# jgkellymit/GENIE-SMEM

Measured on NVIDIA B200. Metric: SMEM reads/sec (BWA-SMEM; LUT/RMI under methods), higher is better.
Workload: dtype u32

## Files before the change

genie_smem_b200/csrc/fm_core.cuh:

```cuda
#pragma once
#include <stdint.h>

#if defined(__CUDACC__)
#define GSM_HD __host__ __device__ __forceinline__
#else
#define GSM_HD inline
#endif

namespace gsm {

struct U4 {
    uint32_t x, y, z, w;
};

struct Half {
    uint32_t c0, c1;
    uint32_t l0, l1, l2;
    uint32_t h0, h1, h2;
};

GSM_HD uint32_t popc32(uint32_t v) {
#if defined(__CUDA_ARCH__)
    return (uint32_t)__popc(v);
#else
    return (uint32_t)__builtin_popcount(v);
#endif
}

GSM_HD void split192(uint32_t p, uint32_t& bucket, uint32_t& r) {
#if defined(__CUDA_ARCH__)
    bucket = __umulhi(p >> 6, 0xAAAAAAABu) >> 1;
#else
    bucket = (p >> 6) / 3u;
#endif
    r = p - bucket * 192u;
}

GSM_HD uint32_t mask_low(uint32_t n) {
#if defined(__CUDA_ARCH__)
    uint32_t m;
    asm("bmsk.clamp.b32 %0, %1, %2;" : "=r"(m) : "r"(0u), "r"(n));
    return m;
#else
    return n >= 32u ? 0xFFFFFFFFu : ((1u << n) - 1u);
#endif
}

GSM_HD uint32_t clamp32(int v) { return (uint32_t)(v < 0 ? 0 : (v > 32 ? 32 : v)); }

struct SymK {
    uint32_t fl, fh;
    uint32_t X, Y;
    uint32_t nz;
};

GSM_HD SymK sym_consts(uint32_t c) {
    SymK k;
    k.fl = 0u - ((c & 1u) ^ 1u);
    k.fh = 0u - (((c >> 1) & 1u) ^ 1u);
    k.X = 0u - (c >> 1);
    k.Y = 0u - (c & (c >> 1));
    k.nz = 0u - (uint32_t)(c != 0u);
    return k;
}

GSM_HD uint32_t half_counts(const Half& v, uint32_t r, const SymK& k, uint32_t g) {
    const int n = (int)r - 96 * (int)g;
    const uint32_t m0 = mask_low(clamp32(n)), m1 = mask_low(clamp32(n - 32)), m2 = mask_low(clamp32(n - 64));
    const uint32_t eq = popc32((v.l0 ^ k.fl) & (v.h0 ^ k.fh) & m0) + popc32((v.l1 ^ k.fl) & (v.h1 ^ k.fh) & m1) +
                        popc32((v.l2 ^ k.fl) & (v.h2 ^ k.fh) & m2);
    const uint32_t lt = popc32(((~v.h0 & (~v.l0 | k.X)) | (~v.l0 & k.Y)) & m0 & k.nz) +
                        popc32(((~v.h1 & (~v.l1 | k.X)) | (~v.l1 & k.Y)) & m1 & k.nz) +
                        popc32(((~v.h2 & (~v.l2 | k.X)) | (~v.l2 & k.Y)) & m2 & k.nz);
    return eq | (lt << 8);
}

GSM_HD void half_header(const Half& v, uint32_t c, uint32_t g, uint32_t& h_eq, uint32_t& h_lt) {
    const uint32_t mine = (c >> 1) == g ? ((c & 1u) ? v.c1 : v.c0) : 0u;
    const uint32_t lt0 = (c >= 1u ? v.c0 : 0u) + (c >= 2u ? v.c1 : 0u);
    const uint32_t lt1 = c == 3u ? v.c0 : 0u;
    h_eq = mine;
    h_lt = g == 0u ? lt0 : lt1;
}

struct StepOut {
    uint32_t lo_new, cnt_new, lt_add;
};

GSM_HD StepOut finish_step(uint32_t eq0, uint32_t eq1, uint32_t ltd, uint32_t P0, uint32_t P1, uint32_t c, uint32_t Cc,
                           uint32_t primary) {
    const uint32_t a0 = P0 > primary ? 1u : 0u;
    const uint32_t a1 = P1 > primary ? 1u : 0u;
    const uint32_t inrange = a1 - a0;
    const uint32_t isA = c == 0u ? 1u : 0u;
    StepOut o;
    o.lo_new = Cc + eq0 - (isA & a0);
    o.cnt_new = (eq1 - eq0) - (isA & inrange);
    o.lt_add = isA ? inrange : ltd;
    return o;
}

GSM_HD void bucket_masks(const Half& h0, const Half& h1, const SymK& k, uint32_t (&E)[6], uint32_t (&T)[6]) {
    const uint32_t L[6] = {h0.l0, h0.l1, h0.l2, h1.l0, h1.l1, h1.l2}, H[6] = {h0.h0, h0.h1, h0.h2, h1.h0, h1.h1, h1.h2};
#if defined(__CUDA_ARCH__)
#pragma unroll
#endif
    for (int w = 0; w < 6; ++w) {
        E[w] = (L[w] ^ k.fl) & (H[w] ^ k.fh);
        T[w] = ((~H[w] & (~L[w] | k.X)) | (~L[w] & k.Y)) & k.nz;
    }
}

GSM_HD uint32_t bucket_counts(const uint32_t (&E)[6], const uint32_t (&T)[6], uint32_t r) {
    uint32_t eq = 0, lt = 0;
#if defined(__CUDA_ARCH__)
#pragma unroll
#endif
    for (int w = 0; w < 6; ++w) {
        const uint32_t m = mask_low(clamp32((int)r - 32 * w));
        eq += popc32(E[w] & m);
        lt += popc32(T[w] & m);
    }
    return eq | (lt << 16);
}

template <typename LoadHalf>
GSM_HD StepOut step_single(LoadHalf load, uint32_t P0, uint32_t P1, uint32_t c, uint32_t Cc, uint32_t primary) {
    const SymK k = sym_consts(c);
    uint32_t b0, r0, b1, r1;
    split192(P0, b0, r0);
    split192(P1, b1, r1);
    uint32_t E[6], T[6];
    const Half a0 = load((uint64_t)b0 * 2), a1 = load((uint64_t)b0 * 2 + 1);
    bucket_masks(a0, a1, k, E, T);
    const uint32_t acc0 = bucket_counts(E, T, r0);
    uint32_t e0, l0, e1, l1;
    half_header(a0, c, 0u, e0, l0);
    half_header(a1, c, 1u, e1, l1);
    const uint32_t eq0 = e0 + e1 + (acc0 & 0xFFFFu), lt0 = l0 + l1 + (acc0 >> 16);
    uint32_t eq1, lt1;
    if (b1 == b0) {
        const uint32_t acc1 = bucket_counts(E, T, r1);
        eq1 = e0 + e1 + (acc1 & 0xFFFFu); lt1 = l0 + l1 + (acc1 >> 16);
    } else {
        const Half c0 = load((uint64_t)b1 * 2), c1 = load((uint64_t)b1 * 2 + 1);
        bucket_masks(c0, c1, k, E, T);
        const uint32_t acc1 = bucket_counts(E, T, r1);
        half_header(c0, c, 0u, e0, l0);
        half_header(c1, c, 1u, e1, l1);
        eq1 = e0 + e1 + (acc1 & 0xFFFFu); lt1 = l0 + l1 + (acc1 >> 16);
    }
    return finish_step(eq0, eq1, lt1 - lt0, P0, P1, c, Cc, primary);
}

template <typename LoadHalf>
GSM_HD uint32_t lf_single(LoadHalf load, uint32_t r, const uint32_t* C, uint32_t primary) {
    uint32_t b, off;
    split192(r, b, off);
    const Half h0 = load((uint64_t)b * 2), h1 = load((uint64_t)b * 2 + 1);
    const uint32_t g = off >= 96u ? 1u : 0u, o = off - 96u * g;
    const Half& hs = g ? h1 : h0;
    const uint32_t lw = o < 32u ? hs.l0 : (o < 64u ? hs.l1 : hs.l2);
    const uint32_t hw = o < 32u ? hs.h0 : (o < 64u ? hs.h1 : hs.h2);
    const uint32_t c = ((lw >> (o & 31u)) & 1u) | (((hw >> (o & 31u)) & 1u) << 1);
    const SymK k = sym_consts(c);
    uint32_t e0, l0, e1, l1;
    half_header(h0, c, 0u, e0, l0);
    half_header(h1, c, 1u, e1, l1);
    const uint32_t acc = half_counts(h0, off, k, 0u) + half_counts(h1, off, k, 1u);
    uint32_t rank = e0 + e1 + (acc & 0xFFu);
    if (c == 0u && r > primary) rank -= 1u;
    return C[c] + rank;
}

GSM_HD uint32_t base_msb(const uint32_t* words, uint32_t pos) { return (words[pos >> 4] >> (30u - 2u * (pos & 15u))) & 3u; }

template <typename LoadW>
GSM_HD uint64_t kmer_code(LoadW load, uint64_t p, uint32_t K) {
    uint64_t w = p >> 4;
    uint32_t sh = 2u * (uint32_t)(p & 15u);
    uint64_t hi = ((uint64_t)load(w) << 32) | (uint64_t)load(w + 1);
    uint64_t v = hi << sh;
    if (sh) v |= (uint64_t)load(w + 2) >> (32u - sh);
    return v >> (64u - 2u * K);
}

}
```

genie_smem_b200/csrc/index_device.cu:

```cuda
#include <cuda_runtime.h>

#include <cub/block/block_reduce.cuh>
#include <cub/block/block_scan.cuh>
#include <cub/device/device_radix_sort.cuh>

#include <algorithm>
#include <cstdint>
#include <cstring>
#include <string>

#include "../../include/genie_smem.h"
#include "fm_core.cuh"
#include "host_common.hpp"

namespace gsm {

#define GSM_CUDA(call)                                                                          \
    do {                                                                                        \
        cudaError_t e__ = (call);                                                               \
        if (e__ != cudaSuccess)                                                                 \
            return fail(GSM_E_CUDA, std::string(#call) + ": " + cudaGetErrorString(e__));       \
    } while (0)

namespace {
// ... 137 lines not shown
            if (u) {
                const unsigned long long o = carry_s + eo;
                out_keys[o] = (unsigned long long)head << 32;
                out_vals[o] = start;
                out_pos[o] = row;
            }
        }
        carry_m = max(carry_m, am);
        carry_s += as;
        __syncthreads();
    }
}

__global__ void __launch_bounds__(BT) k_round_keys(unsigned long long* keys, const uint32_t* vals, const uint32_t* rank, uint64_t m, uint64_t h,
                                                   uint64_t N) {
    const uint64_t k = (uint64_t)blockIdx.x * BT + threadIdx.x;
    if (k >= m) return;
    const uint64_t p = (uint64_t)vals[k] + h;
    uint32_t r;
    if (p <= N) r = rank[p];
    else r = (p - N) <= VIRT ? VIRT - (uint32_t)(p - N) : 0u;
    keys[k] |= (unsigned long long)r;
}

__global__ void __launch_bounds__(BT) k_bwt_planes(const uint32_t* sa1, const uint32_t* text, uint64_t n_rows, uint64_t n_buckets, uint32_t* buckets,
                                                   uint4* bucket_cnt, uint32_t* primary) {
    const uint32_t lane = threadIdx.x & 31u;
    const uint64_t warp0 = ((uint64_t)blockIdx.x * BT + threadIdx.x) >> 5;
    const uint64_t n_warps = ((uint64_t)gridDim.x * BT) >> 5;
    for (uint64_t b = warp0; b < n_buckets; b += n_warps) {
        uint32_t c0 = 0, c1 = 0, c2 = 0, c3 = 0;
        uint32_t* w = buckets + b * 16;
#pragma unroll
        for (int g = 0; g < 2; ++g)
#pragma unroll
            for (int mth = 0; mth < 3; ++mth) {
                const uint64_t r = b * GSM_BUCKET_SYMS + 96 * g + 32 * mth + lane;
                const bool valid = r < n_rows;
                uint32_t c = 0;
                if (valid) {
                    const uint32_t s1 = __ldg(sa1 + r);
                    if (s1 == 1u) *primary = (uint32_t)r;
                    else c = text_base(text, (uint64_t)s1 - 2u);
                }
                const uint32_t lo = __ballot_sync(0xFFFFFFFFu, valid && (c & 1u));
                const uint32_t hi = __ballot_sync(0xFFFFFFFFu, valid && (c >> 1));
                const uint32_t vm = __ballot_sync(0xFFFFFFFFu, valid);
                const uint32_t n3 = __popc(lo & hi), n2 = __popc(hi & ~lo), n1 = __popc(lo & ~hi);
                c3 += n3; c2 += n2; c1 += n1; c0 += __popc(vm) - n1 - n2 - n3;
                if (lane == 0) {
                    w[8 * g + 2 + mth] = lo;
                    w[8 * g + 5 + mth] = hi;
                }
            }
        if (lane == 0) bucket_cnt[b] = make_uint4(c0, c1, c2, c3);
    }
}

struct Add4 {
    __device__ __forceinline__ uint4 operator()(const uint4& a, const uint4& b) const { return make_uint4(a.x + b.x, a.y + b.y, a.z + b.z, a.w + b.w); }
};

__global__ void __launch_bounds__(BT) k_cnt_reduce(const uint4* cnt, uint64_t n, uint4* tile_sum) {
    using Reduce = cub::BlockReduce<uint4, BT>;
    __shared__ typename Reduce::TempStorage tmp;
    const uint64_t t0 = (uint64_t)blockIdx.x * TILE;
    uint4 acc = make_uint4(0, 0, 0, 0);
    for (int s = 0; s < SUBTILES; ++s) {
        const uint64_t k = t0 + (uint64_t)s * BT + threadIdx.x;
        if (k < n) acc = Add4()(acc, cnt[k]);
    }
    acc = Reduce(tmp).Reduce(acc, Add4());
    if (threadIdx.x == 0) tile_sum[blockIdx.x] = acc;
}

__global__ void __launch_bounds__(1024) k_cnt_top(uint4* tile_sum, uint64_t n_tiles, uint4* total) {
    using Scan = cub::BlockScan<uint4, 1024>;
    __shared__ typename Scan::TempStorage tmp;
    uint4 carry = make_uint4(0, 0, 0, 0);
    for (uint64_t base = 0; base < n_tiles; base += 1024) {
        const uint64_t t = base + threadIdx.x;
        const uint4 v = t < n_tiles ? tile_sum[t] : make_uint4(0, 0, 0, 0);
        uint4 ex, agg;
        Scan(tmp).ExclusiveScan(v, ex, make_uint4(0, 0, 0, 0), Add4(), agg);
        if (t < n_tiles) tile_sum[t] = Add4()(ex, carry);
        carry = Add4()(carry, agg);
        __syncthreads();
    }
    if (threadIdx.x == 0) *total = carry;
}

__global__ void __launch_bounds__(BT) k_cnt_apply(const uint4* cnt, uint64_t n, const uint4* tile_pre, uint32_t* buckets) {
    using Scan = cub::BlockScan<uint4, BT>;
    __shared__ typename Scan::TempStorage tmp;
    const uint64_t t0 = (uint64_t)blockIdx.x * TILE;
    uint4 carry = tile_pre[blockIdx.x];
    for (int s = 0; s < SUBTILES; ++s) {
        const uint64_t k = t0 + (uint64_t)s * BT + threadIdx.x;
        const uint4 v = k < n ? cnt[k] : make_uint4(0, 0, 0, 0);
        uint4 ex, agg;
        Scan(tmp).ExclusiveScan(v, ex, make_uint4(0, 0, 0, 0), Add4(), agg);
        if (k < n) {
            const uint4 p = Add4()(ex, carry);
            uint32_t* w = buckets + k * 16;
            w[0] = p.x; w[1] = p.y; w[8] = p.z; w[9] = p.w;
        }
        carry = Add4()(carry, agg);
        __syncthreads();
    }
}

struct Carve {
    uint8_t* base;
    uint64_t off = 0;
    explicit Carve(void* b) : base((uint8_t*)b) {}
    template <typename T>
    T* take(uint64_t count) {
        off = (off + 255) & ~255ull;
        T* p = base ? (T*)(base + off) : nullptr;
        off += count * sizeof(T);
        return p;
    }
};

struct Plan {
    unsigned long long *k0, *k1, *tile_off, *scalars;
    uint32_t *v0, *v1, *p0, *p1, *rank, *rtext, *tile_max, *tile_cnt;
    uint4 *bucket_cnt, *cnt_tiles;
    void* cub_tmp;
    uint64_t cub_bytes, total;
};

uint64_t cub_sort_bytes(uint64_t n) {
    size_t bytes = 0;
    cub::DoubleBuffer<unsigned long long> dk(nullptr, nullptr);
    cub::DoubleBuffer<uint32_t> dv(nullptr, nullptr);
    cub::DeviceRadixSort::SortPairs(nullptr, bytes, dk, dv, (uint64_t)n, 0, 64, (cudaStream_t)0);
    return (uint64_t)bytes;
// ... 180 lines not shown
```

genie_smem_b200/csrc/index_host.cpp:

```cpp
#include <algorithm>
#include <cstdint>
#include <cstdio>
#include <cstdlib>
#include <cstring>
#include <new>
#include <string>
#include <thread>
#include <vector>

#include "../../include/genie_smem.h"
#include "host_common.hpp"

namespace gsm {

thread_local std::string g_last_error;

int fail(int code, const std::string& msg) {
    g_last_error = msg;
    return code;
}

namespace {

template <typename Ch>
// ... 79 lines not shown
        } else {
            for (int32_t i = 0; i < n1; ++i) SA1[s1[i]] = i;
        }

        buckets(true);
        for (int32_t i = 1, j = 0; i < n; ++i)
            if (is_lms(i)) s1[j++] = i;
        for (int32_t i = 0; i < n1; ++i) SA1[i] = s1[SA1[i]];
        std::fill(SA + n1, SA + n, -1);
        for (int32_t i = n1 - 1; i >= 0; --i) {
            int32_t j = SA[i];
            SA[i] = -1;
            SA[--bkt[s[j]]] = j;
        }
        induce_l();
        induce_s();
    }
};

}

void suffix_sort(const uint8_t* sym, int32_t* SA, int32_t n) {
    Sais<uint8_t> top;
    top.s = sym; top.SA = SA; top.n = n; top.K = 5;
    top.run();
}

void pack_buckets(const uint8_t* bwt, uint64_t n, std::vector<uint32_t>& out) {
    uint64_t nb = n / GSM_BUCKET_SYMS + 1;
    out.assign(nb * 16, 0);
    uint32_t run[4] = {0, 0, 0, 0};
    for (uint64_t b = 0; b < nb; ++b) {
        uint32_t* w = &out[b * 16];
        w[0] = run[0]; w[1] = run[1]; w[8] = run[2]; w[9] = run[3];
        uint64_t base = b * GSM_BUCKET_SYMS;
        for (int g = 0; g < 2; ++g)
            for (int m = 0; m < 3; ++m) {
                uint32_t lo = 0, hi = 0;
                for (int t = 0; t < 32; ++t) {
                    uint64_t r = base + 96 * g + 32 * m + t;
                    if (r >= n) break;
                    uint32_t c = bwt[r];
                    run[c]++;
                    lo |= (c & 1u) << t;
                    hi |= (c >> 1) << t;
                }
                w[8 * g + 2 + m] = lo;
                w[8 * g + 5 + m] = hi;
            }
    }
}

}

using namespace gsm;

struct gsm_index {
    uint64_t n_bases = 0;
    uint64_t n = 0;
    std::vector<uint8_t> codes;
    std::vector<int32_t> sa0;
    std::vector<uint32_t> fwd, rev;
    uint32_t count[4] = {0, 0, 0, 0};
    uint32_t C[5] = {0, 0, 0, 0, 0};
    uint32_t primary_fwd = 0, primary_rev = 0;
    bool has_rev = false;
};

static int decode_bases(const char* bases, uint64_t n_bases, std::vector<uint8_t>& codes, uint32_t count[4]) {
    static int8_t map[256];
    static bool init = false;
    if (!init) {
        memset(map, -1, sizeof(map));
        map[(int)'A'] = 0; map[(int)'C'] = 1; map[(int)'G'] = 2; map[(int)'T'] = 3;
        init = true;
    }
    codes.resize(n_bases);
    for (uint64_t i = 0; i < n_bases; ++i) {
        int8_t c = map[(uint8_t)bases[i]];
        if (c < 0) return fail(GSM_E_INVALID, "non-ACGT base at offset " + std::to_string(i));
        codes[i] = (uint8_t)c;
        count[c]++;
// ... 208 lines not shown
```

genie_smem_b200/csrc/sweep_device.cuh:

```cuda
#pragma once
#include <cuda_runtime.h>

#include "sweep_logic.cuh"

namespace gsm {

constexpr int SWEEP_THREADS = 128;
constexpr int SWEEP_LPR = 2;
constexpr int SWEEP_GROUPS = SWEEP_THREADS / SWEEP_LPR;
constexpr int SWEEP_CAP = 12;
constexpr int SWEEP_MIN_BLOCKS = 8;

constexpr uint32_t MEMS_ORDERED = 0x80000000u;
constexpr uint32_t MEMS_PICKED = 0x40000000u;
constexpr uint32_t MEMS_COUNT = 0x3FFFFFFFu;

struct SweepArgs {
    const uint4* fwd;
    const uint4* rev;
    IndexMeta meta;
    const uint4* reads;
    const uint32_t* chunk_off;
    const uint32_t* len;
    uint32_t n_reads;
// ... 4 lines not shown
    uint32_t seed_K;
    uint4* mem_pool;
    unsigned long long mem_cap;
    uint32_t* mem_off;
    uint32_t* mem_cnt;
    uint4* scratch;
    unsigned long long* counters;
    const uint32_t* sa;
    const uint32_t* text;
    uint32_t n_bases;
};

extern __shared__ uint4 g_sweep_smem[];

__device__ __forceinline__ Half ldg_half(const uint4* halves_base, size_t half_index) {
    Half h;
    asm volatile("ld.global.nc.v8.u32 {%0,%1,%2,%3,%4,%5,%6,%7}, [%8];"
                 : "=r"(h.c0), "=r"(h.c1), "=r"(h.l0), "=r"(h.l1), "=r"(h.l2), "=r"(h.h0), "=r"(h.h1), "=r"(h.h2)
                 : "l"(halves_base + half_index * 2));
    return h;
}

__device__ __forceinline__ StepOut pair_step(const uint4* __restrict__ bk, uint32_t P0, uint32_t P1, uint32_t ch, uint32_t Cc,
                                             uint32_t primary, uint32_t g, bool active) {
    constexpr uint32_t FULLM = 0xFFFFFFFFu;
    uint32_t b0, r0, b1, r1;
    split192(P0, b0, r0);
    split192(P1, b1, r1);
    Half v0 = Half{0, 0, 0, 0, 0, 0, 0, 0}, v1;
    if (active) v0 = ldg_half(bk, (size_t)b0 * 2 + g);
    v1 = v0;
    if (active && b1 != b0) v1 = ldg_half(bk, (size_t)b1 * 2 + g);
    const SymK k = sym_consts(ch);
    uint32_t packed = half_counts(v0, r0, k, g) | (half_counts(v1, r1, k, g) << 16);
    uint32_t he0, hl0, he1, hl1;
    half_header(v0, ch, g, he0, hl0);
    half_header(v1, ch, g, he1, hl1);
    uint32_t A = he0, B = he1, D = hl1 - hl0;
    packed += __shfl_xor_sync(FULLM, packed, 1);
    A += __shfl_xor_sync(FULLM, A, 1);
    B += __shfl_xor_sync(FULLM, B, 1);
    D += __shfl_xor_sync(FULLM, D, 1);
    const uint32_t eq0 = A + (packed & 0xFFu);
    const uint32_t eq1 = B + ((packed >> 16) & 0xFFu);
    const uint32_t ltd = D + ((packed >> 24) & 0xFFu) - ((packed >> 8) & 0xFFu);
    return finish_step(eq0, eq1, ltd, P0, P1, ch, Cc, primary);
}

__device__ __forceinline__ uint4 ldg_seed(const uint4* p) {
    uint4 v;
    asm volatile("ld.global.nc.v4.u32 {%0,%1,%2,%3}, [%4];" : "=r"(v.x), "=r"(v.y), "=r"(v.z), "=r"(v.w) : "l"(p));
    return v;
}

__device__ __forceinline__ uint32_t spread4(uint32_t x) { return ((x * 0x01004010u) | (x >> 6)) & 0x03030303u; }

struct DevSweepCtx {
    const SweepArgs& a;
    uint32_t cand0;
    uint32_t bytes0;
    uint32_t words0;
    uint4* stage;
    uint4* spill;
    uint32_t g, gmask, gbase;

    __device__ __forceinline__ bool fetch(uint32_t& rid, uint32_t& L) {
        unsigned long long r = 0;
        if (g == 0) r = atomicAdd(&a.counters[3], 1ull);
        r = __shfl_sync(gmask, r, gbase);
        if (r >= a.n_reads) return false;
        rid = (uint32_t)r;
        L = __ldg(a.len + rid);
        const uint32_t off = __ldg(a.chunk_off + rid);
        const uint32_t nch = (L + 63u) >> 6;
        uint4* dst = g_sweep_smem + (bytes0 >> 4);
        __syncwarp(gmask);
        for (uint32_t c = g; c < nch; c += SWEEP_LPR) {
            const uint4 v = __ldg(a.reads + (size_t)off + c);
            g_sweep_smem[(words0 >> 2) + c] = v;
// ... 52 lines not shown
    const uint32_t pair_in_block = threadIdx.x >> 1;
    const uint32_t pair_u4 = SWEEP_CAP + a.read_u4 + a.pack_u4;
    const uint32_t p0 = pair_in_block * pair_u4;
    const size_t gp = (size_t)blockIdx.x * SWEEP_GROUPS + pair_in_block;
    DevSweepCtx ctx{a, p0, (p0 + SWEEP_CAP) * 16u, (p0 + SWEEP_CAP + a.read_u4) * 4u, a.scratch + gp * 2 * a.max_len,
                    a.scratch + gp * 2 * a.max_len + a.max_len, g, 3u << (lane & ~1u), lane & ~1u};
    Sweeper<DevSweepCtx> sw;
    for (;;) {
        const bool need = sw.next(ctx, a.meta);
        if (!__any_sync(0xFFFFFFFFu, need)) break;
        const bool is_seed = need && sw.pending_seed();
        const bool is_step = need && !is_seed;
        uint4 se = make_uint4(0u, 0u, 0u, 0u);
        if (is_seed) se = ldg_seed(a.seed_tab + sw.P0);
        const bool rev = sw.on_reverse();
        const StepOut r = pair_step(rev ? a.rev : a.fwd, sw.P0, sw.P0 + sw.cnt, sw.ch, a.meta.C[sw.ch & 3u],
                                    rev ? a.meta.prim_r : a.meta.prim_f, g, is_step);
        if (is_step) sw.consume(ctx, a.meta, r);
        else if (is_seed) sw.consume_seed(ctx, a.meta, SeedEntry{se.x, se.y, se.z, se.w});
    }
}

constexpr int SWEEP1_THREADS = 128;
constexpr int SWEEP1_CAP = 8;
constexpr int SWEEP1_MIN_BLOCKS = 7;

struct LanePartial {
    uint32_t eq0, lt0;
    bool have;
};

template <bool PAIRED>
__device__ __forceinline__ bool lane_step(const uint4* __restrict__ fwd, const uint4* __restrict__ rev, bool use_rev, uint32_t P0, uint32_t P1,
                                          uint32_t ch, uint32_t Cc, uint32_t primary, bool active, LanePartial& part, StepOut& out) {
    constexpr uint32_t FULLM = 0xFFFFFFFFu;
    uint32_t b0, r0, b1, r1;
    split192(P0, b0, r0);
    split192(P1, b1, r1);
    const bool second = part.have;
    const uint32_t b = second ? b1 : b0;
    Half a0 = Half{0, 0, 0, 0, 0, 0, 0, 0}, a1 = a0;
    if (PAIRED) {
        const uint32_t g = threadIdx.x & 1u;
        const uint32_t mine = (active ? 1u : 0u) | (use_rev ? 2u : 0u);
        const uint32_t pb = __shfl_xor_sync(FULLM, b, 1);
        const uint32_t theirs = __shfl_xor_sync(FULLM, mine, 1);
#pragma unroll
        for (uint32_t r = 0; r < 2u; ++r) {
            const bool own = g == r;
            const uint32_t bb = own ? b : pb, fl = own ? mine : theirs;
            Half h = Half{0, 0, 0, 0, 0, 0, 0, 0};
            if (fl & 1u) h = ldg_half((fl & 2u) ? rev : fwd, (size_t)bb * 2 + (own ? 0u : 1u));
            Half o;
            o.c0 = __shfl_xor_sync(FULLM, h.c0, 1); o.c1 = __shfl_xor_sync(FULLM, h.c1, 1);
            o.l0 = __shfl_xor_sync(FULLM, h.l0, 1); o.l1 = __shfl_xor_sync(FULLM, h.l1, 1); o.l2 = __shfl_xor_sync(FULLM, h.l2, 1);
            o.h0 = __shfl_xor_sync(FULLM, h.h0, 1); o.h1 = __shfl_xor_sync(FULLM, h.h1, 1); o.h2 = __shfl_xor_sync(FULLM, h.h2, 1);
            if (own) { a0 = h; a1 = o; }
        }
    } else if (active) {
        const uint4* bk = use_rev ? rev : fwd;
        a0 = ldg_half(bk, (size_t)b * 2);
        a1 = ldg_half(bk, (size_t)b * 2 + 1);
    }
    const SymK k = sym_consts(ch);
    uint32_t E[6], T[6];
    bucket_masks(a0, a1, k, E, T);
    const uint32_t accA = bucket_counts(E, T, second ? r1 : r0);
    const uint32_t accB = bucket_counts(E, T, r1);
    uint32_t e0, l0, e1, l1;
    half_header(a0, ch, 0u, e0, l0);
    half_header(a1, ch, 1u, e1, l1);
    const uint32_t he = e0 + e1, hl = l0 + l1;
    if (!active) return false;
    if (!second && b1 != b0) {
        part.eq0 = he + (accA & 0xFFFFu);
        part.lt0 = hl + (accA >> 16);
        part.have = true;
        return false;
    }
    const uint32_t eq0 = second ? part.eq0 : he + (accA & 0xFFFFu);
    const uint32_t eq1 = he + ((second ? accA : accB) & 0xFFFFu);
    const uint32_t ltd = second ? hl + (accA >> 16) - part.lt0 : (accB >> 16) - (accA >> 16);
    part.have = false;
    out = finish_step(eq0, eq1, ltd, P0, P1, ch, Cc, primary);
    return true;
}

__device__ __noinline__ void hand_over_long(const uint4* sp, uint32_t n, uint4* dst) {
    constexpr uint32_t FULLM = 0xFFFFFFFFu;
    const uint32_t lane = threadIdx.x & 31u;
    uint4 v0 = make_uint4(0u, 0u, 0u, 0u), v1 = v0;
    if (lane < n) v0 = __ldcg(sp + lane);
    if (lane + 32u < n) v1 = __ldcg(sp + lane + 32u);
    const uint32_t prev0 = __shfl_up_sync(FULLM, v0.w, 1);
    const uint32_t last0 = __shfl_sync(FULLM, v0.w, 31);
    uint32_t prev1 = __shfl_up_sync(FULLM, v1.w, 1);
    if (lane == 0u) prev1 = last0;
    const unsigned long long heads =
        (unsigned long long)__ballot_sync(FULLM, lane < n && (lane == 0u || v0.w != prev0)) |
        ((unsigned long long)__ballot_sync(FULLM, lane + 32u < n && v1.w != prev1) << 32);
    uint32_t* seg = reinterpret_cast<uint32_t*>(dst);
#pragma unroll
    for (int half = 0; half < 2; ++half) {
        const uint32_t x = lane + 32u * half;
        if (x < n) {
            const uint4 v = half ? v1 : v0;
            const unsigned long long upto = heads & (~0ull >> (63u - x));
            const uint32_t s0 = 63u - (uint32_t)__clzll((long long)upto);
            const unsigned long long above = x == 63u ? 0ull : heads & (~0ull << (x + 1u));
            const uint32_t s1 = above ? (uint32_t)__ffsll((long long)above) - 1u : n;
            const uint32_t d = s0 + (s1 - 1u - x);
            seg[d] = v.x; seg[n + d] = v.y; seg[2u * n + d] = v.z; seg[3u * n + d] = v.w;
        }
    }
}
// ... 122 lines not shown
            } else if (n <= SOA_MAX) {
                hand_over_long(sp, n, a.mem_pool + off);
            } else {
                for (uint32_t k = lane; k < n; k += 32u) a.mem_pool[off + k] = __ldcg(sp + k);
            }
        }
        if (fin_n != NO_FIN) {
            a.mem_off[fin_rid] = fits ? (uint32_t)my_off : 0u;
            a.mem_cnt[fin_rid] = fits ? (fin_n | (fin_n <= SOA_MAX ? MEMS_ORDERED : 0u) | (fin_n >= 1u && fin_n <= 32u ? MEMS_PICKED : 0u)) : 0u;
            fin_n = NO_FIN;
        }
    }
};

constexpr uint32_t SWEEP1_SMEM_MAX_LEN = 1024;
constexpr uint64_t SWEEP1_LONG_SCRATCH = 4ull << 30;

__host__ __device__ inline uint32_t sweep1_lane_u4(uint32_t max_len, bool long_reads) {
    return SWEEP1_CAP + (long_reads ? 0u : (max_len + 63u) / 64u + 1u);
}
inline size_t sweep1_smem_bytes(uint32_t max_len, bool long_reads) {
    return (size_t)SWEEP1_THREADS * sweep1_lane_u4(max_len, long_reads) * sizeof(uint4) + 16;
}

template <bool LONG, bool UNIQ, int MB = SWEEP1_MIN_BLOCKS, bool STATS = false, bool PAIRED = false>
__global__ void __launch_bounds__(SWEEP1_THREADS, MB) k_sweep1(const SweepArgs a) {
    using Ctx = DevSweepCtx1<LONG, UNIQ>;
    const uint32_t lane_u4 = sweep1_lane_u4(a.max_len, LONG);
    const uint32_t p0 = threadIdx.x * lane_u4;
    const size_t gl = (size_t)blockIdx.x * SWEEP1_THREADS + threadIdx.x;
    Ctx ctx{a, p0, (p0 + SWEEP1_CAP) * 4u, a.scratch + gl * 2 * a.max_len, a.scratch + gl * 2 * a.max_len + a.max_len, nullptr, 0u, Ctx::NO_FIN};
    Sweeper<Ctx> sw;
    LanePartial part{0u, 0u, false};
    uint32_t n_it = 0, n_step = 0, n_seed = 0, n_text = 0;
    for (;;) {
        ctx.flush_finished();
        const bool need = sw.next(ctx, a.meta);
        if (__any_sync(0xFFFFFFFFu, ctx.fin_n != Ctx::NO_FIN)) ctx.flush_finished();
        if (!__any_sync(0xFFFFFFFFu, need)) break;
        const bool is_seed = need && sw.pending_seed();
        const bool is_word = UNIQ && need && sw.pending_word();
        const bool is_cmp = UNIQ && need && sw.pending_cmp();
        const bool is_step = need && !is_seed && !is_word && !is_cmp;
        if (STATS) { n_it++; n_step += is_step; n_seed += is_seed; n_text += is_word || is_cmp; }
        uint4 se = make_uint4(0u, 0u, 0u, 0u);
        if (is_seed) se = ldg_seed(a.seed_tab + sw.P0);
        uint32_t wv = 0u, matched = 0u;
        if (UNIQ && is_word) wv = __ldg(a.sa + sw.aux);
        if (UNIQ && is_cmp) {
            matched = ctx.match_forward(sw.cmp_text(), sw.cmp_read());
            const uint32_t mx = sw.cmp_max(a.n_bases);
            matched = matched < mx ? matched : mx;
        }
        const bool rev = sw.on_reverse();
        StepOut r;
        const bool stepped = lane_step<PAIRED>(a.fwd, a.rev, rev, sw.P0, sw.P0 + sw.cnt, sw.ch, a.meta.C[sw.ch & 3u],
                                               rev ? a.meta.prim_r : a.meta.prim_f, is_step, part, r);
        if (stepped) sw.consume(ctx, a.meta, r);
        else if (is_seed) sw.consume_seed(ctx, a.meta, SeedEntry{se.x, se.y, se.z, se.w});
        else if (UNIQ && is_word) sw.consume_word(ctx, a.meta, wv);
        else if (UNIQ && is_cmp) sw.consume_cmp(ctx, a.meta, matched);
    }
    if (STATS) {
        atomicAdd(&a.counters[4], (unsigned long long)n_it);
        atomicAdd(&a.counters[5], (unsigned long long)n_step);
        atomicAdd(&a.counters[6], (unsigned long long)n_seed);
        atomicAdd(&a.counters[7], (unsigned long long)n_text);
    }
}

__host__ __device__ inline uint32_t sweep_pack_u4(uint32_t max_len) { return (max_len + 63u) / 64u; }

inline size_t sweep_smem_bytes(uint32_t max_len) {
    return (size_t)SWEEP_GROUPS * (SWEEP_CAP + sweep_read_u4(max_len) + sweep_pack_u4(max_len)) * sizeof(uint4) + 16;
}

}
```

genie_smem_b200/engine.py:

```python
import ctypes as C

import numpy as np
import torch

from . import _capi as capi
from .ingest import Contigs

RECORD_DTYPE = np.dtype([("read_id", "<u4"), ("qstart", "<u2"), ("qend", "<u2"), ("sa_lo", "<u4"), ("sa_hi", "<u4")])
HIT_DTYPE = np.dtype([("record", "<u4"), ("contig", "<u4"), ("offset", "<u4"), ("flags", "<u4")])
CHAIN_DTYPE = np.dtype([("slot", "<u4"), ("contig", "<u4"), ("rbeg", "<u4"), ("rend", "<u4"), ("q", "<u4"), ("weight", "<u4"),
                        ("n_seeds", "<u4"), ("reserved", "<u4")])
_BASES = np.frombuffer(b"ACGT", dtype=np.uint8)


class BaseError(KeyError, ValueError):
    """A read or reference holds a character outside ACGT (the reference raises KeyError there,
    SMEM/ExactMatch.py:139; SURVEY 8b asks for ValueError up front -- this is both)."""


def _ptr(t):
    return C.c_void_p(t.data_ptr()) if t is not None else C.c_void_p(0)


def _stream():
# ... 64 lines not shown

    def pack(self, with_sa=True, with_text=True):
        i = self.info
        fwd = np.zeros(i.n_buckets * 16, np.uint32)
        rev = np.zeros(i.n_buckets * 16, np.uint32) if i.has_reverse else None
        sa = np.zeros(i.n_rows, np.uint32) if with_sa else None
        text = np.zeros(i.text_words + 2, np.uint32) if with_text else None
        capi.check(capi.lib.gsm_index_pack(self._h, fwd.ctypes.data, rev.ctypes.data if rev is not None else None,
                                           sa.ctypes.data if sa is not None else None, text.ctypes.data if text is not None else None))
        return fwd, rev, sa, text

    def close(self):
        if self._h is not None:
            capi.lib.gsm_index_free(self._h)
            self._h = None

    def __del__(self):
        try:
            self.close()
        except Exception:
            pass


def _to_dev(a, device):
    if a is None:
        return None
    a = np.asarray(a)
    if not a.flags.writeable:
        a = np.array(a)
    t = torch.from_numpy(a.view(np.int32))
    return t.to(device, non_blocking=False)


class PackedIndex:

    FIELDS = ("n_bases", "n_rows", "n_buckets", "bucket_bytes", "text_words", "primary_fwd", "primary_rev", "has_reverse")

    def __init__(self, info, fwd, rev, sa, text):
        self.info, self.fwd, self.rev, self.sa, self.text = info, fwd, rev, sa, text

    @classmethod
    def from_host(cls, host: HostIndex, with_sa=True, with_text=True):
        return cls(host.info, *host.pack(with_sa, with_text))

    @classmethod
    def from_device(cls, index, with_sa=True, with_text=True):
        def grab(t):
            return None if t is None else t.cpu().numpy().view(np.uint32)
        return cls(index.info, grab(index.fwd), grab(index.rev), grab(index.sa) if with_sa else None, grab(index.text) if with_text else None)

    def save(self, directory):
        import json as _json
        import os as _os
        _os.makedirs(directory, exist_ok=True)
        meta = {k: int(getattr(self.info, k)) for k in self.FIELDS}
        meta["count"] = [int(x) for x in self.info.count]
        meta["C"] = [int(x) for x in self.info.C]
        meta["format"] = "genie_smem_b200 packed index v1 (64-byte buckets = two 32-byte halves)"
        for name in ("fwd", "rev", "sa", "text"):
            a = getattr(self, name)
            if a is not None:
                np.save(_os.path.join(directory, name + ".npy"), a)
        with open(_os.path.join(directory, "meta.json"), "w") as f:
            _json.dump(meta, f, indent=1)

    @classmethod
    def load(cls, directory, mmap=True):
        import json as _json
        import os as _os
        with open(_os.path.join(directory, "meta.json")) as f:
            meta = _json.load(f)
        info = capi.IndexInfo()
        for k in cls.FIELDS:
            setattr(info, k, meta[k])
        for c in range(4):
            info.count[c] = meta["count"][c]
        for c in range(5):
            info.C[c] = meta["C"][c]
        arrs = []
        for name in ("fwd", "rev", "sa", "text"):
            p = _os.path.join(directory, name + ".npy")
            arrs.append(np.load(p, mmap_mode="r" if mmap else None) if _os.path.exists(p) else None)
        return cls(info, *arrs)


class IndexFile:

    MAGIC = b"GSMIDX02"
    ALIGN = 4096

    @staticmethod
    def _sections(index, lut, rmi):
        def host(t):
            return None if t is None else t.detach().cpu().numpy()
        sec = [("fwd", host(index.fwd)), ("rev", host(index.rev)), ("sa", host(index.sa)), ("text", host(index.text)),
               ("ssa", host(getattr(index, "ssa", None))), ("seed_table", host(getattr(index, "seed_table", None))), ("lut", host(lut))]
        if rmi is not None:
            sec += [("rmi_params", host(rmi.params)), ("rmi_probe", host(rmi.probe))]
        return [(n, a) for n, a in sec if a is not None]

    @classmethod
    def save(cls, path, index, lut=None, lut_K=0, rmi=None, contigs=None):
        import json as _json
        import zlib
        info = {k: int(getattr(index.info, k)) for k in PackedIndex.FIELDS}
        info["count"] = [int(x) for x in index.info.count]
        info["C"] = [int(x) for x in index.info.C]
        head = {"format": "genie_smem_b200 index file v2", "info": info, "seed_K": int(getattr(index, "seed_K", 0) or 0),
                "sa_sample": int(getattr(index, "sa_sample", 0) or 0), "lut_K": int(lut_K) if lut is not None else 0, "rmi": None, "sections": []}
        if rmi is not None:
            head["rmi"] = {"K": rmi.K, "level_sizes": [int(x) for x in rmi.level_sizes],
                           "none_rows": [int(x) for x in rmi.none_rows] if rmi.none_rows is not None else None,
                           "max_err": float(getattr(rmi, "max_err", -1.0))}
        secs = cls._sections(index, lut, rmi)
        if contigs is not None:
            if contigs.n_bases != int(index.info.n_bases):
                raise ValueError(f"contigs cover {contigs.n_bases} bases, the index {int(index.info.n_bases)}")
            head["contigs"] = list(contigs.names)
            secs.append(("contig_start", contigs.start))
        for n, a in secs:
            head["sections"].append({"name": n, "dtype": str(a.dtype), "shape": list(a.shape), "offset": 0, "nbytes": int(a.nbytes),
                                     "crc32": zlib.crc32(memoryview(np.ascontiguousarray(a)).cast("B")) & 0xFFFFFFFF})
        blob = _json.dumps(head).encode()
        room = ((len(blob) + 16 + 64 * len(secs) + cls.ALIGN - 1) // cls.ALIGN) * cls.ALIGN
        off = room
        for d in head["sections"]:
            d["offset"] = off
            off += ((d["nbytes"] + cls.ALIGN - 1) // cls.ALIGN) * cls.ALIGN
        blob = _json.dumps(head).encode()
        assert 16 + len(blob) <= room
        with open(path, "wb") as f:
            f.write(cls.MAGIC)
            f.write(np.uint64(len(blob)).tobytes())
            f.write(blob)
            for d, (n, a) in zip(head["sections"], secs):
                f.seek(d["offset"])
                np.ascontiguousarray(a).tofile(f)
            f.truncate(off)
        return off

    @classmethod
    def header(cls, path):
        import json as _json
        with open(path, "rb") as f:
            if f.read(8) != cls.MAGIC:
                raise ValueError(f"{path}: not a genie_smem_b200 index file")
            n = int(np.frombuffer(f.read(8), np.uint64)[0])
            return _json.loads(f.read(n).decode())

    @classmethod
    def load(cls, path, device="cuda", verify=False):
        import zlib
        require_cuda()
        head = cls.header(path)
        arrs = {}
        for d in head["sections"]:
            a = np.memmap(path, mode="r", dtype=np.dtype(d["dtype"]), offset=d["offset"], shape=tuple(d["shape"]))
            if verify and (zlib.crc32(memoryview(a).cast("B")) & 0xFFFFFFFF) != d["crc32"]:
                raise ValueError(f"{path}: section {d['name']} is corrupt (CRC-32 mismatch)")
            arrs[d["name"]] = a
        info = capi.IndexInfo()
        for k in PackedIndex.FIELDS:
            setattr(info, k, head["info"][k])
        for c in range(4):
            info.count[c] = head["info"]["count"][c]
        for c in range(5):
            info.C[c] = head["info"]["C"][c]
        dev = torch.device(device)

        def up(name):
            a = arrs.get(name)
            return None if a is None else torch.from_numpy(np.array(a)).to(dev)
        index = DeviceIndex.__new__(DeviceIndex)
        index.device, index.info, index.build_stats = dev, info, None
        index.fwd, index.rev, index.sa, index.text = up("fwd"), up("rev"), up("sa"), up("text")
        if "ssa" in arrs:
            index.ssa, index.sa_sample = up("ssa"), head["sa_sample"]
        if "seed_table" in arrs:
            index.seed_table, index.seed_K = up("seed_table"), head["seed_K"]
        index._bind()
        if "contigs" in head:
            index.set_contigs(Contigs(head["contigs"], np.array(arrs["contig_start"])))
        lut = up("lut")
        rmi = None
        if head["rmi"] is not None:
            p = np.array(arrs["rmi_params"])
            rmi = RmiParams(head["rmi"]["K"], head["rmi"]["level_sizes"], p[:, 0], p[:, 1], dev)
            rmi.max_err = head["rmi"]["max_err"]
            if head["rmi"]["none_rows"] is not None:
                rows = np.asarray(head["rmi"]["none_rows"], np.uint32)
                rmi.none_rows = rows
                rmi.c.none_rows = rows.ctypes.data_as(capi.u32p)
                rmi.c.n_none_rows = len(rows)
            if "rmi_probe" in arrs:
                rmi.probe = up("rmi_probe")
                rmi.c.probe = rmi.probe.data_ptr()
        return index, lut, head["lut_K"], rmi


class DeviceIndex:

    contigs = None
    _contig_start = None

# ... 1206 lines not shown
```

Measured before the change: 216.6 million.

## Anchor each bucket half at its first row so rank queries load one half

Changes the packed bucket format so the second 32-byte half stores occurrence counts anchored at its own midpoint. Rank queries for G/T can then count backward from the midpoint when the position is past it, and the unpaired lane step loads only the half or halves it actually needs. The goal is to cut global-memory traffic per backward-extension step. In exchange, the index format version changes, older files are converted at load time, the popcount masking logic becomes more complex, and a new half-load counter is added.

```diff
diff --git a/genie_smem_b200/csrc/fm_core.cuh b/genie_smem_b200/csrc/fm_core.cuh
--- a/genie_smem_b200/csrc/fm_core.cuh
+++ b/genie_smem_b200/csrc/fm_core.cuh
@@ -52,6 +52,7 @@
     uint32_t fl, fh;
     uint32_t X, Y;
     uint32_t nz;
+    uint32_t mid;
 };
 
 GSM_HD SymK sym_consts(uint32_t c) {
@@ -61,26 +62,42 @@
     k.X = 0u - (c >> 1);
     k.Y = 0u - (c & (c >> 1));
     k.nz = 0u - (uint32_t)(c != 0u);
+    k.mid = 0u - (c >> 1);
     return k;
 }
 
-GSM_HD uint32_t half_counts(const Half& v, uint32_t r, const SymK& k, uint32_t g) {
-    const int n = (int)r - 96 * (int)g;
-    const uint32_t m0 = mask_low(clamp32(n)), m1 = mask_low(clamp32(n - 32)), m2 = mask_low(clamp32(n - 64));
-    const uint32_t eq = popc32((v.l0 ^ k.fl) & (v.h0 ^ k.fh) & m0) + popc32((v.l1 ^ k.fl) & (v.h1 ^ k.fh) & m1) +
-                        popc32((v.l2 ^ k.fl) & (v.h2 ^ k.fh) & m2);
-    const uint32_t lt = popc32(((~v.h0 & (~v.l0 | k.X)) | (~v.l0 & k.Y)) & m0 & k.nz) +
-                        popc32(((~v.h1 & (~v.l1 | k.X)) | (~v.l1 & k.Y)) & m1 & k.nz) +
-                        popc32(((~v.h2 & (~v.l2 | k.X)) | (~v.l2 & k.Y)) & m2 & k.nz);
-    return eq | (lt << 8);
-}
-
-GSM_HD void half_header(const Half& v, uint32_t c, uint32_t g, uint32_t& h_eq, uint32_t& h_lt) {
-    const uint32_t mine = (c >> 1) == g ? ((c & 1u) ? v.c1 : v.c0) : 0u;
-    const uint32_t lt0 = (c >= 1u ? v.c0 : 0u) + (c >= 2u ? v.c1 : 0u);
-    const uint32_t lt1 = c == 3u ? v.c0 : 0u;
-    h_eq = mine;
-    h_lt = g == 0u ? lt0 : lt1;
+GSM_HD uint32_t halves_needed(uint32_t c, uint32_t lo, uint32_t hi) {
+    return (c >= 2u && lo >= 96u ? 0u : 1u) | (c < 2u && hi <= 96u ? 0u : 2u);
+}
+
+GSM_HD void half_anchor(const Half& v, uint32_t g, uint32_t c, uint32_t b, uint32_t& eq, uint32_t& lt) {
+    const bool mine = (c >> 1) == g;
+    const uint32_t e = (c & 1u) ? v.c1 : v.c0;
+    const uint32_t l = g == 0u ? (c != 0u ? v.c0 : 0u) : b * 192u + 96u - v.c1 - (c == 2u ? v.c0 : 0u);
+    eq = mine ? e : 0u;
+    lt = mine ? l : 0u;
+}
+
+GSM_HD void bucket_anchor(const Half& h0, const Half& h1, uint32_t c, uint32_t b, uint32_t& eq, uint32_t& lt) {
+    uint32_t e0, l0, e1, l1;
+    half_anchor(h0, 0u, c, b, e0, l0);
+    half_anchor(h1, 1u, c, b, e1, l1);
+    eq = e0 + e1;
+    lt = l0 + l1;
+}
+
+GSM_HD uint32_t plane_mask(uint32_t r, int w, uint32_t neg) { return mask_low(clamp32((int)r - 32 * w)) ^ neg; }
+
+GSM_HD void half_rank(const Half& v, uint32_t g, const SymK& k, uint32_t r, uint32_t& eq, uint32_t& lt) {
+    const uint32_t neg = g == 0u ? k.mid : 0u;
+    const uint32_t m0 = plane_mask(r, 3 * (int)g, neg), m1 = plane_mask(r, 3 * (int)g + 1, neg), m2 = plane_mask(r, 3 * (int)g + 2, neg);
+    const uint32_t e = popc32((v.l0 ^ k.fl) & (v.h0 ^ k.fh) & m0) + popc32((v.l1 ^ k.fl) & (v.h1 ^ k.fh) & m1) +
+                       popc32((v.l2 ^ k.fl) & (v.h2 ^ k.fh) & m2);
+    const uint32_t l = popc32(((~v.h0 & (~v.l0 | k.X)) | (~v.l0 & k.Y)) & m0 & k.nz) +
+                       popc32(((~v.h1 & (~v.l1 | k.X)) | (~v.l1 & k.Y)) & m1 & k.nz) +
+                       popc32(((~v.h2 & (~v.l2 | k.X)) | (~v.l2 & k.Y)) & m2 & k.nz);
+    eq = (e ^ neg) - neg;
+    lt = (l ^ neg) - neg;
 }
 
 struct StepOut {
@@ -111,17 +128,26 @@
     }
 }
 
-GSM_HD uint32_t bucket_counts(const uint32_t (&E)[6], const uint32_t (&T)[6], uint32_t r) {
+GSM_HD uint32_t anchored_packed(const uint32_t (&E)[6], const uint32_t (&T)[6], uint32_t neg, uint32_t r, uint32_t& d) {
     uint32_t eq = 0, lt = 0;
 #if defined(__CUDA_ARCH__)
 #pragma unroll
 #endif
     for (int w = 0; w < 6; ++w) {
-        const uint32_t m = mask_low(clamp32((int)r - 32 * w));
-        eq += popc32(E[w] & m);
-        lt += popc32(T[w] & m);
+        const uint32_t n = w < 3 ? neg : 0u;
+        const uint32_t m = plane_mask(r, w, n);
+        eq += popc32((E[w] ^ n) & m);
+        lt += popc32((T[w] ^ n) & m);
     }
+    d = neg & ((r < 96u ? r : 96u) - 96u);
     return eq | (lt << 16);
+}
+
+GSM_HD void anchored_counts(const uint32_t (&E)[6], const uint32_t (&T)[6], uint32_t neg, uint32_t r, uint32_t& eq, uint32_t& lt) {
+    uint32_t d;
+    const uint32_t p = anchored_packed(E, T, neg, r, d);
+    eq = (p & 0xFFFFu) + d;
+    lt = (p >> 16) + d;
 }
 
 template <typename LoadHalf>
@@ -133,23 +159,17 @@
     uint32_t E[6], T[6];
     const Half a0 = load((uint64_t)b0 * 2), a1 = load((uint64_t)b0 * 2 + 1);
     bucket_masks(a0, a1, k, E, T);
-    const uint32_t acc0 = bucket_counts(E, T, r0);
-    uint32_t e0, l0, e1, l1;
-    half_header(a0, c, 0u, e0, l0);
-    half_header(a1, c, 1u, e1, l1);
-    const uint32_t eq0 = e0 + e1 + (acc0 & 0xFFFFu), lt0 = l0 + l1 + (acc0 >> 16);
-    uint32_t eq1, lt1;
-    if (b1 == b0) {
-        const uint32_t acc1 = bucket_counts(E, T, r1);
-        eq1 = e0 + e1 + (acc1 & 0xFFFFu); lt1 = l0 + l1 + (acc1 >> 16);
-    } else {
+    uint32_t ae, al, eq0, lt0, eq1, lt1;
+    bucket_anchor(a0, a1, c, b0, ae, al);
+    anchored_counts(E, T, k.mid, r0, eq0, lt0);
+    eq0 += ae; lt0 += al;
+    if (b1 != b0) {
         const Half c0 = load((uint64_t)b1 * 2), c1 = load((uint64_t)b1 * 2 + 1);
         bucket_masks(c0, c1, k, E, T);
-        const uint32_t acc1 = bucket_counts(E, T, r1);
-        half_header(c0, c, 0u, e0, l0);
-        half_header(c1, c, 1u, e1, l1);
-        eq1 = e0 + e1 + (acc1 & 0xFFFFu); lt1 = l0 + l1 + (acc1 >> 16);
+        bucket_anchor(c0, c1, c, b1, ae, al);
     }
+    anchored_counts(E, T, k.mid, r1, eq1, lt1);
+    eq1 += ae; lt1 += al;
     return finish_step(eq0, eq1, lt1 - lt0, P0, P1, c, Cc, primary);
 }
 
@@ -164,11 +184,11 @@
     const uint32_t hw = o < 32u ? hs.h0 : (o < 64u ? hs.h1 : hs.h2);
     const uint32_t c = ((lw >> (o & 31u)) & 1u) | (((hw >> (o & 31u)) & 1u) << 1);
     const SymK k = sym_consts(c);
-    uint32_t e0, l0, e1, l1;
-    half_header(h0, c, 0u, e0, l0);
-    half_header(h1, c, 1u, e1, l1);
-    const uint32_t acc = half_counts(h0, off, k, 0u) + half_counts(h1, off, k, 1u);
-    uint32_t rank = e0 + e1 + (acc & 0xFFu);
+    uint32_t ae, al, e0, l0, e1, l1;
+    bucket_anchor(h0, h1, c, b, ae, al);
+    half_rank(h0, 0u, k, off, e0, l0);
+    half_rank(h1, 1u, k, off, e1, l1);
+    uint32_t rank = ae + e0 + e1;
     if (c == 0u && r > primary) rank -= 1u;
     return C[c] + rank;
 }
diff --git a/genie_smem_b200/csrc/index_device.cu b/genie_smem_b200/csrc/index_device.cu
--- a/genie_smem_b200/csrc/index_device.cu
+++ b/genie_smem_b200/csrc/index_device.cu
@@ -193,7 +193,7 @@
         uint32_t c0 = 0, c1 = 0, c2 = 0, c3 = 0;
         uint32_t* w = buckets + b * 16;
 #pragma unroll
-        for (int g = 0; g < 2; ++g)
+        for (int g = 0; g < 2; ++g) {
 #pragma unroll
             for (int mth = 0; mth < 3; ++mth) {
                 const uint64_t r = b * GSM_BUCKET_SYMS + 96 * g + 32 * mth + lane;
@@ -214,6 +214,8 @@
                     w[8 * g + 5 + mth] = hi;
                 }
             }
+            if (g == 0 && lane == 0) { w[8] = c2; w[9] = c3; }
+        }
         if (lane == 0) bucket_cnt[b] = make_uint4(c0, c1, c2, c3);
     }
 }
@@ -264,7 +266,7 @@
         if (k < n) {
             const uint4 p = Add4()(ex, carry);
             uint32_t* w = buckets + k * 16;
-            w[0] = p.x; w[1] = p.y; w[8] = p.z; w[9] = p.w;
+            w[0] = p.x; w[1] = p.y; w[8] += p.z; w[9] += p.w;
         }
         carry = Add4()(carry, agg);
         __syncthreads();
diff --git a/genie_smem_b200/csrc/index_host.cpp b/genie_smem_b200/csrc/index_host.cpp
--- a/genie_smem_b200/csrc/index_host.cpp
+++ b/genie_smem_b200/csrc/index_host.cpp
@@ -135,9 +135,9 @@
     uint32_t run[4] = {0, 0, 0, 0};
     for (uint64_t b = 0; b < nb; ++b) {
         uint32_t* w = &out[b * 16];
-        w[0] = run[0]; w[1] = run[1]; w[8] = run[2]; w[9] = run[3];
         uint64_t base = b * GSM_BUCKET_SYMS;
-        for (int g = 0; g < 2; ++g)
+        for (int g = 0; g < 2; ++g) {
+            w[8 * g] = run[2 * g]; w[8 * g + 1] = run[2 * g + 1];
             for (int m = 0; m < 3; ++m) {
                 uint32_t lo = 0, hi = 0;
                 for (int t = 0; t < 32; ++t) {
@@ -151,6 +151,7 @@
                 w[8 * g + 2 + m] = lo;
                 w[8 * g + 5 + m] = hi;
             }
+        }
     }
 }
 
diff --git a/genie_smem_b200/csrc/sweep_device.cuh b/genie_smem_b200/csrc/sweep_device.cuh
--- a/genie_smem_b200/csrc/sweep_device.cuh
+++ b/genie_smem_b200/csrc/sweep_device.cuh
@@ -60,19 +60,16 @@
     v1 = v0;
     if (active && b1 != b0) v1 = ldg_half(bk, (size_t)b1 * 2 + g);
     const SymK k = sym_consts(ch);
-    uint32_t packed = half_counts(v0, r0, k, g) | (half_counts(v1, r1, k, g) << 16);
-    uint32_t he0, hl0, he1, hl1;
-    half_header(v0, ch, g, he0, hl0);
-    half_header(v1, ch, g, he1, hl1);
-    uint32_t A = he0, B = he1, D = hl1 - hl0;
-    packed += __shfl_xor_sync(FULLM, packed, 1);
+    uint32_t ae0, al0, ae1, al1, e0, l0, e1, l1;
+    half_anchor(v0, g, ch, b0, ae0, al0);
+    half_anchor(v1, g, ch, b1, ae1, al1);
+    half_rank(v0, g, k, r0, e0, l0);
+    half_rank(v1, g, k, r1, e1, l1);
+    uint32_t A = ae0 + e0, B = ae1 + e1, D = (al1 + l1) - (al0 + l0);
     A += __shfl_xor_sync(FULLM, A, 1);
     B += __shfl_xor_sync(FULLM, B, 1);
     D += __shfl_xor_sync(FULLM, D, 1);
-    const uint32_t eq0 = A + (packed & 0xFFu);
-    const uint32_t eq1 = B + ((packed >> 16) & 0xFFu);
-    const uint32_t ltd = D + ((packed >> 24) & 0xFFu) - ((packed >> 8) & 0xFFu);
-    return finish_step(eq0, eq1, ltd, P0, P1, ch, Cc, primary);
+    return finish_step(A, B, D, P0, P1, ch, Cc, primary);
 }
 
 __device__ __forceinline__ uint4 ldg_seed(const uint4* p) {
@@ -191,19 +188,22 @@
 
 template <bool PAIRED>
 __device__ __forceinline__ bool lane_step(const uint4* __restrict__ fwd, const uint4* __restrict__ rev, bool use_rev, uint32_t P0, uint32_t P1,
-                                          uint32_t ch, uint32_t Cc, uint32_t primary, bool active, LanePartial& part, StepOut& out) {
+                                          uint32_t ch, uint32_t Cc, uint32_t primary, bool active, LanePartial& part, StepOut& out,
+                                          uint32_t& n_halves) {
     constexpr uint32_t FULLM = 0xFFFFFFFFu;
     uint32_t b0, r0, b1, r1;
     split192(P0, b0, r0);
     split192(P1, b1, r1);
     const bool second = part.have;
     const uint32_t b = second ? b1 : b0;
+    const uint32_t rlo = second ? r1 : r0, rhi = b1 == b0 ? r1 : rlo;
     Half a0 = Half{0, 0, 0, 0, 0, 0, 0, 0}, a1 = a0;
     if (PAIRED) {
         const uint32_t g = threadIdx.x & 1u;
         const uint32_t mine = (active ? 1u : 0u) | (use_rev ? 2u : 0u);
         const uint32_t pb = __shfl_xor_sync(FULLM, b, 1);
         const uint32_t theirs = __shfl_xor_sync(FULLM, mine, 1);
+        n_halves += active ? 2u : 0u;
 #pragma unroll
         for (uint32_t r = 0; r < 2u; ++r) {
             const bool own = g == r;
@@ -216,30 +216,32 @@
             o.h0 = __shfl_xor_sync(FULLM, h.h0, 1); o.h1 = __shfl_xor_sync(FULLM, h.h1, 1); o.h2 = __shfl_xor_sync(FULLM, h.h2, 1);
             if (own) { a0 = h; a1 = o; }
         }
-    } else if (active) {
+    } else {
+        const uint32_t need = active ? halves_needed(ch, rlo, rhi) : 0u;
+        n_halves += popc32(need);
         const uint4* bk = use_rev ? rev : fwd;
-        a0 = ldg_half(bk, (size_t)b * 2);
-        a1 = ldg_half(bk, (size_t)b * 2 + 1);
+        if (active) {
+            a0 = ldg_half(bk, (size_t)b * 2 + (need == 2u ? 1u : 0u));
+            a1 = ldg_half(bk, (size_t)b * 2 + (need == 1u ? 0u : 1u));
+        }
     }
     const SymK k = sym_consts(ch);
     uint32_t E[6], T[6];
     bucket_masks(a0, a1, k, E, T);
-    const uint32_t accA = bucket_counts(E, T, second ? r1 : r0);
-    const uint32_t accB = bucket_counts(E, T, r1);
-    uint32_t e0, l0, e1, l1;
-    half_header(a0, ch, 0u, e0, l0);
-    half_header(a1, ch, 1u, e1, l1);
-    const uint32_t he = e0 + e1, hl = l0 + l1;
+    uint32_t dA, dB, he, hl;
+    const uint32_t accA = anchored_packed(E, T, k.mid, rlo, dA);
+    const uint32_t accB = anchored_packed(E, T, k.mid, r1, dB);
+    bucket_anchor(a0, a1, ch, b, he, hl);
     if (!active) return false;
     if (!second && b1 != b0) {
-        part.eq0 = he + (accA & 0xFFFFu);
-        part.lt0 = hl + (accA >> 16);
+        part.eq0 = he + dA + (accA & 0xFFFFu);
+        part.lt0 = hl + dA + (accA >> 16);
         part.have = true;
         return false;
     }
-    const uint32_t eq0 = second ? part.eq0 : he + (accA & 0xFFFFu);
-    const uint32_t eq1 = he + ((second ? accA : accB) & 0xFFFFu);
-    const uint32_t ltd = second ? hl + (accA >> 16) - part.lt0 : (accB >> 16) - (accA >> 16);
+    const uint32_t eq0 = second ? part.eq0 : he + dA + (accA & 0xFFFFu);
+    const uint32_t eq1 = second ? he + dA + (accA & 0xFFFFu) : he + dB + (accB & 0xFFFFu);
+    const uint32_t ltd = second ? hl + dA + (accA >> 16) - part.lt0 : dB + (accB >> 16) - dA - (accA >> 16);
     part.have = false;
     out = finish_step(eq0, eq1, ltd, P0, P1, ch, Cc, primary);
     return true;
@@ -428,7 +430,7 @@
     Ctx ctx{a, p0, (p0 + SWEEP1_CAP) * 4u, a.scratch + gl * 2 * a.max_len, a.scratch + gl * 2 * a.max_len + a.max_len, nullptr, 0u, Ctx::NO_FIN};
     Sweeper<Ctx> sw;
     LanePartial part{0u, 0u, false};
-    uint32_t n_it = 0, n_step = 0, n_seed = 0, n_text = 0;
+    uint32_t n_it = 0, n_step = 0, n_seed = 0, n_text = 0, n_half = 0;
     for (;;) {
         ctx.flush_finished();
         const bool need = sw.next(ctx, a.meta);
@@ -451,7 +453,7 @@
         const bool rev = sw.on_reverse();
         StepOut r;
         const bool stepped = lane_step<PAIRED>(a.fwd, a.rev, rev, sw.P0, sw.P0 + sw.cnt, sw.ch, a.meta.C[sw.ch & 3u],
-                                               rev ? a.meta.prim_r : a.meta.prim_f, is_step, part, r);
+                                               rev ? a.meta.prim_r : a.meta.prim_f, is_step, part, r, n_half);
         if (stepped) sw.consume(ctx, a.meta, r);
         else if (is_seed) sw.consume_seed(ctx, a.meta, SeedEntry{se.x, se.y, se.z, se.w});
         else if (UNIQ && is_word) sw.consume_word(ctx, a.meta, wv);
@@ -462,6 +464,7 @@
         atomicAdd(&a.counters[5], (unsigned long long)n_step);
         atomicAdd(&a.counters[6], (unsigned long long)n_seed);
         atomicAdd(&a.counters[7], (unsigned long long)n_text);
+        atomicAdd(&a.counters[1], (unsigned long long)n_half);
     }
 }
 
diff --git a/genie_smem_b200/engine.py b/genie_smem_b200/engine.py
--- a/genie_smem_b200/engine.py
+++ b/genie_smem_b200/engine.py
@@ -120,9 +120,22 @@
     return t.to(device, non_blocking=False)
 
 
+def midpoint_anchored(buckets):
+    if buckets is None:
+        return None
+    a = np.asarray(buckets)
+    w = np.array(a.view(np.uint32).reshape(-1, 16))
+    lo, hi = w[:, 2:5], w[:, 5:8]
+    w[:, 8] += np.bitwise_count(hi & ~lo).sum(axis=1, dtype=np.uint32)
+    w[:, 9] += np.bitwise_count(hi & lo).sum(axis=1, dtype=np.uint32)
+    return w.reshape(-1).view(a.dtype)
+
+
 class PackedIndex:
 
     FIELDS = ("n_bases", "n_rows", "n_buckets", "bucket_bytes", "text_words", "primary_fwd", "primary_rev", "has_reverse")
+    FORMAT = "genie_smem_b200 packed index v2 (64-byte buckets = two 32-byte halves, each anchored at its first row)"
+    FORMAT_V1 = "genie_smem_b200 packed index v1 (64-byte buckets = two 32-byte halves)"
 
     def __init__(self, info, fwd, rev, sa, text):
         self.info, self.fwd, self.rev, self.sa, self.text = info, fwd, rev, sa, text
@@ -144,7 +157,7 @@
         meta = {k: int(getattr(self.info, k)) for k in self.FIELDS}
         meta["count"] = [int(x) for x in self.info.count]
         meta["C"] = [int(x) for x in self.info.C]
-        meta["format"] = "genie_smem_b200 packed index v1 (64-byte buckets = two 32-byte halves)"
+        meta["format"] = self.FORMAT
         for name in ("fwd", "rev", "sa", "text"):
             a = getattr(self, name)
             if a is not None:
@@ -169,12 +182,18 @@
         for name in ("fwd", "rev", "sa", "text"):
             p = _os.path.join(directory, name + ".npy")
             arrs.append(np.load(p, mmap_mode="r" if mmap else None) if _os.path.exists(p) else None)
+        if meta.get("format") == cls.FORMAT_V1:
+            arrs[0], arrs[1] = midpoint_anchored(arrs[0]), midpoint_anchored(arrs[1])
+        elif meta.get("format") != cls.FORMAT:
+            raise ValueError(f"{directory}: unknown packed index format {meta.get('format')!r}")
         return cls(info, *arrs)
 
 
 class IndexFile:
 
-    MAGIC = b"GSMIDX02"
+    MAGIC = b"GSMIDX03"
+    MAGIC_V2 = b"GSMIDX02"
+    FORMAT = "genie_smem_b200 index file v3"
     ALIGN = 4096
 
     @staticmethod
@@ -194,7 +213,7 @@
         info = {k: int(getattr(index.info, k)) for k in PackedIndex.FIELDS}
         info["count"] = [int(x) for x in index.info.count]
         info["C"] = [int(x) for x in index.info.C]
-        head = {"format": "genie_smem_b200 index file v2", "info": info, "seed_K": int(getattr(index, "seed_K", 0) or 0),
+        head = {"format": cls.FORMAT, "info": info, "seed_K": int(getattr(index, "seed_K", 0) or 0),
                 "sa_sample": int(getattr(index, "sa_sample", 0) or 0), "lut_K": int(lut_K) if lut is not None else 0, "rmi": None, "sections": []}
         if rmi is not None:
             head["rmi"] = {"K": rmi.K, "level_sizes": [int(x) for x in rmi.level_sizes],
@@ -231,10 +250,13 @@
     def header(cls, path):
         import json as _json
         with open(path, "rb") as f:
-            if f.read(8) != cls.MAGIC:
+            magic = f.read(8)
+            if magic not in (cls.MAGIC, cls.MAGIC_V2):
                 raise ValueError(f"{path}: not a genie_smem_b200 index file")
             n = int(np.frombuffer(f.read(8), np.uint64)[0])
-            return _json.loads(f.read(n).decode())
+            head = _json.loads(f.read(n).decode())
+            head["midpoint_anchored"] = magic == cls.MAGIC
+            return head
 
     @classmethod
     def load(cls, path, device="cuda", verify=False):
@@ -258,6 +280,8 @@
 
         def up(name):
             a = arrs.get(name)
+            if a is not None and name in ("fwd", "rev") and not head["midpoint_anchored"]:
+                return torch.from_numpy(midpoint_anchored(a)).to(dev)
             return None if a is None else torch.from_numpy(np.array(a)).to(dev)
         index = DeviceIndex.__new__(DeviceIndex)
         index.device, index.info, index.build_stats = dev, info, None
```

Result: slower. 194.6 million (median of 6 runs) (-10.2%).
